# NagabhushanSN95/SimpleNeRF

Hardware: AMD Instinct MI355X
Metric: rays/sec (coarse+fine, 128+128 samples) (higher is better)
Workload: dtype f32; 1 GPU; headline: 1024 rays/GPU x (128 coarse + 128 fine -> 256 merged) samples, 8x256 coarse+fine MLPs, LLFF fern NDC rays, eval; rays_per_gpu=1024, samples=128+128, parallelism=ray-shard x1

## Files before the change

### simplenerf_amd/csrc/clock_stamp.h

```cpp
#pragma once
#ifdef SNERF_CLOCK_STAMP
#define SNERF_STAMP_DEFINE(name)                                                                                          \
    static __device__ unsigned long long name##_stamps[2 * 8192];                                                         \
    extern "C" __attribute__((weak)) int snerf_debug_clock_stamps_##name(unsigned long long* host, int pairs) {           \
        return (int)hipMemcpyFromSymbol(host, HIP_SYMBOL(name##_stamps), sizeof(unsigned long long) * 2 * (pairs < 8192 ? pairs : 8192)); \
    }
#define SNERF_STAMP_BEGIN() \
    const unsigned long long stamp_t0 = __builtin_amdgcn_s_memtime(), stamp_r0 = __builtin_amdgcn_s_memrealtime()
#define SNERF_STAMP_END(name)                                                                       \
    do {                                                                                            \
        if (threadIdx.x == 0) {                                                                     \
            name##_stamps[2 * (blockIdx.x & 8191)] = __builtin_amdgcn_s_memtime() - stamp_t0;       \
            name##_stamps[2 * (blockIdx.x & 8191) + 1] = __builtin_amdgcn_s_memrealtime() - stamp_r0; \
        }                                                                                           \
    } while (0)
#else
#define SNERF_STAMP_DEFINE(name)
#define SNERF_STAMP_BEGIN() do {} while (0)
#define SNERF_STAMP_END(name) do {} while (0)
#endif
```

### simplenerf_amd/csrc/composite.hip

```cpp
#include "composite_device.h"

namespace {

template <int C, bool RESAMPLE = false>
__global__ void __launch_bounds__(256) composite_kernel(CompositeArgs a) {
    extern __shared__ __attribute__((aligned(16))) float lds[];
    const int lane = snerf::lane_id();
    const long long ray = (long long)blockIdx.x * 4 + (threadIdx.x >> 6);
    if (ray >= a.num_rays) return;
    const int s = a.s;
    float* mine = RESAMPLE ? lds + (size_t)(threadIdx.x >> 6) * (s + snerf::resample_scratch_floats(s, a.s_f)) : nullptr;
    composite_ray<C, RESAMPLE>(a, ray, a.z + ray * s, a.sigma + ray * s, a.rgb + ray * s * 3, mine,
                               RESAMPLE ? a.z_fine + ray * (s + a.s_f) : nullptr, lane);
}

template <int C, bool RESAMPLE = false>
void launch(const CompositeArgs& a, hipStream_t stream) {
    const long long blocks = (a.num_rays + 3) / 4;
    const size_t lds_bytes = RESAMPLE ? 4 * sizeof(float) * (size_t)(a.s + snerf::resample_scratch_floats(a.s, a.s_f)) : 0;
    hipLaunchKernelGGL((composite_kernel<C, RESAMPLE>), dim3((unsigned)blocks), dim3(256), lds_bytes, stream, a);
}

template <bool RESAMPLE>
void launch_for_samples(const CompositeArgs& a, hipStream_t st) {
    const int c = (a.s + 63) / 64;
    switch (c) {
        case 1: launch<1, RESAMPLE>(a, st); break;
        case 2: launch<2, RESAMPLE>(a, st); break;
        case 3: launch<3, RESAMPLE>(a, st); break;
        case 4: launch<4, RESAMPLE>(a, st); break;
        case 5: case 6: launch<6, RESAMPLE>(a, st); break;
        case 7: case 8: launch<8, RESAMPLE>(a, st); break;
        default: launch<16, RESAMPLE>(a, st); break;
    }
}


struct CompositeBwdArgs {
    const float* sigma; const float* rgb; const float* z; const float* march_dirs; const float* rays_o; const float* rays_d;
    const float* g_rgb; const float* g_acc; const float* g_depth; const float* g_depth_ndc;
    float* d_sigma; float* d_rgb;
    long long num_rays; int s; int ndc; int white;
};

template <int C>
__global__ void __launch_bounds__(256) composite_backward_kernel(CompositeBwdArgs a) {
    const int lane = snerf::lane_id();
    const long long ray = (long long)blockIdx.x * 4 + (threadIdx.x >> 6);
    if (ray >= a.num_rays) return;
    const int s = a.s;
    const float* zr = a.z + ray * s;
    const float* sr = a.sigma + ray * s;
    const float* cr = a.rgb + ray * s * 3;
    const int j0 = lane * C;
    float z[C + 1], sg[C], col[C][3];
#pragma unroll
    for (int c = 0; c < C; ++c) {
        const int j = j0 + c;
        const bool in = j < s;
        z[c] = in ? zr[j] : 0.0f;
        sg[c] = in ? sr[j] : 0.0f;
#pragma unroll
        for (int k = 0; k < 3; ++k) col[c][k] = in ? cr[3 * j + k] : 0.0f;
    }
    const float far_cap = a.ndc ? 1.0f : 1e10f;
    z[C] = __shfl_down(z[0], 1, 64);
    if (j0 + C >= s) z[C] = far_cap;
#pragma unroll
    for (int c = 0; c < C; ++c)
        if (j0 + c == s - 1) z[c + 1] = far_cap;
    const float* md = a.march_dirs + ray * 3;
    const float norm = sqrtf((md[0] * md[0] + md[1] * md[1]) + md[2] * md[2]);

    float alpha[C], delta[C], keep = 1.0f;
#pragma unroll
    for (int c = 0; c < C; ++c) {
        const bool in = j0 + c < s;
        delta[c] = (z[c + 1] - z[c]) * norm;
        alpha[c] = in ? 1.0f - expf(-sg[c] * delta[c]) : 0.0f;
        keep *= in ? (1.0f - alpha[c]) + 1e-10f : 1.0f;
    }
    const float incl = snerf::wave_inclusive_mul(keep);
    float trans = __shfl_up(incl, 1, 64);
    if (lane == 0) trans = 1.0f;
    float T[C], w[C], acc = 0.0f, dzm = 0.0f;
#pragma unroll
    for (int c = 0; c < C; ++c) {
        T[c] = trans;
        w[c] = alpha[c] * trans;
        trans *= (1.0f - alpha[c]) + 1e-10f;
        acc += w[c];
        dzm += w[c] * z[c];
    }
    acc = snerf::wave_sum(acc);
    dzm = snerf::wave_sum(dzm);
    const float inv = __fdiv_rn(1.0f, acc + 1e-6f);
    const float depth_march = dzm * inv;
    float zd[C];
    float depth = depth_march;
    if (a.ndc) {
        const float oz = a.rays_o[ray * 3 + 2], dzw = a.rays_d[ray * 3 + 2];
        const float tn = __fdiv_rn(-(1.0f + oz), dzw);
        const float scale = __fdiv_rn(oz + tn * dzw, dzw);
        float dw = 0.0f;
#pragma unroll
        for (int c = 0; c < C; ++c) {
            const float cst = (z[c] == 1.0f) ? 1e-3f : 0.0f;
            zd[c] = scale * (__fdiv_rn(1.0f, (1.0f - z[c]) + cst) - 1.0f) + tn;
            dw += w[c] * zd[c];
        }
        depth = snerf::wave_sum(dw) * inv;
    } else {
#pragma unroll
        for (int c = 0; c < C; ++c) zd[c] = z[c];
    }
    const float gr = a.g_rgb ? a.g_rgb[ray * 3 + 0] : 0.0f;
    const float gg = a.g_rgb ? a.g_rgb[ray * 3 + 1] : 0.0f;
    const float gb = a.g_rgb ? a.g_rgb[ray * 3 + 2] : 0.0f;
    float gacc = a.g_acc ? a.g_acc[ray] : 0.0f;
    if (a.white) gacc -= (gr + gg) + gb;
    const float gdep = (a.g_depth ? a.g_depth[ray] : 0.0f) * inv;
    const float gdn = (a.ndc && a.g_depth_ndc ? a.g_depth_ndc[ray] : 0.0f) * inv;

    float g[C], local = 0.0f;
#pragma unroll
    for (int c = 0; c < C; ++c) {
        g[c] = ((gr * col[c][0] + gg * col[c][1]) + gb * col[c][2]) + gacc + gdep * (zd[c] - depth) + gdn * (z[c] - depth_march);
        local += g[c] * w[c];
    }
    const float suffix_incl = snerf::wave_suffix_add(local);
    float after = __shfl_down(suffix_incl, 1, 64);
    if (lane == 63) after = 0.0f;
#pragma unroll
    for (int c = C - 1; c >= 0; --c) {
        const int j = j0 + c;
        if (j < s) {
            const float u = (1.0f - alpha[c]) + 1e-10f;
            const float dalpha = g[c] * T[c] - __fdiv_rn(after, u);
            a.d_sigma[ray * s + j] = dalpha * (delta[c] * (1.0f - alpha[c]));
            a.d_rgb[(ray * s + j) * 3 + 0] = w[c] * gr;
            a.d_rgb[(ray * s + j) * 3 + 1] = w[c] * gg;
            a.d_rgb[(ray * s + j) * 3 + 2] = w[c] * gb;
        }
        after += g[c] * w[c];
    }
}

template <int C>
void launch_bwd(const CompositeBwdArgs& a, hipStream_t stream) {
    const long long blocks = (a.num_rays + 3) / 4;
    hipLaunchKernelGGL(composite_backward_kernel<C>, dim3((unsigned)blocks), dim3(256), 0, stream, a);
}

}

extern "C" int snerf_composite(const float* sigma, const float* rgb, const float* depths, const float* march_dirs,
                               const float* rays_o, const float* rays_d, long long num_rays, int num_samples, int ndc,
                               int white_bkgd, float* out_rgb, float* out_acc, float* out_alpha, float* out_visibility,
                               float* out_weights, float* out_depth, float* out_depth_var, float* out_depth_ndc,
                               float* out_depth_var_ndc, snerf_stream_t stream) {
    SNERF_REQUIRE(sigma && rgb && depths && march_dirs, "composite: NULL input");
    SNERF_REQUIRE(out_rgb && out_acc && out_depth && out_depth_var, "composite: NULL required output");
    SNERF_REQUIRE(!ndc || (rays_o && rays_d && out_depth_ndc && out_depth_var_ndc),
                  "composite: ndc needs world rays and the *_ndc outputs");
    SNERF_REQUIRE(num_rays >= 0 && num_samples >= 1, "composite: bad sizes n=%lld S=%d", num_rays, num_samples);
    if (num_samples > 64 * 16)
        return snerf::fail(SNERF_E_UNSUPPORTED, "composite: at most 1024 samples per ray (got %d)", num_samples);
    if (num_rays == 0) return SNERF_OK;
    if ((num_rays + 3) / 4 > 0x7fffffffLL) return snerf::fail(SNERF_E_UNSUPPORTED, "composite: too many rays in one call");
    CompositeArgs a{sigma, rgb, depths, march_dirs, rays_o, rays_d, out_rgb, out_acc, out_alpha, out_visibility,
                    out_weights, out_depth, out_depth_var, out_depth_ndc, out_depth_var_ndc, num_rays, num_samples,
                    ndc, white_bkgd, 0, nullptr, nullptr};
    launch_for_samples<false>(a, (hipStream_t)stream);
    return snerf::check_launch("composite");
}

namespace snerf {
int composite_resample(const float* sigma, const float* rgb, const float* depths, const float* march_dirs, const float* rays_o,
                       const float* rays_d, long long num_rays, int num_samples, int ndc, int white_bkgd, float* out_rgb,
                       float* out_acc, float* out_alpha, float* out_visibility, float* out_weights, float* out_depth,
                       float* out_depth_var, float* out_depth_ndc, float* out_depth_var_ndc, int num_fine, const float* u,
                       float* depths_fine, hipStream_t stream) {
    SNERF_REQUIRE(sigma && rgb && depths && march_dirs && depths_fine, "composite_resample: NULL input");
    SNERF_REQUIRE(out_rgb && out_acc && out_depth && out_depth_var, "composite_resample: NULL required output");
    SNERF_REQUIRE(!ndc || (rays_o && rays_d && out_depth_ndc && out_depth_var_ndc),
                  "composite_resample: ndc needs world rays and the *_ndc outputs");
    if (num_samples < 3 || num_fine < 1 || num_samples > 64 * 16 || (num_rays + 3) / 4 > 0x7fffffffLL ||
        4 * sizeof(float) * (size_t)(num_samples + resample_scratch_floats(num_samples, num_fine)) > 64 * 1024)
        return fail(SNERF_E_UNSUPPORTED, "composite_resample: %d + %d samples not built as one kernel", num_samples, num_fine);
    if (num_rays == 0) return SNERF_OK;
    CompositeArgs a{sigma, rgb, depths, march_dirs, rays_o, rays_d, out_rgb, out_acc, out_alpha, out_visibility,
                    out_weights, out_depth, out_depth_var, out_depth_ndc, out_depth_var_ndc, num_rays, num_samples,
                    ndc, white_bkgd, num_fine, u, depths_fine};
    launch_for_samples<true>(a, stream);
    return check_launch("composite_resample");
}
}

extern "C" int snerf_composite_backward(const float* sigma, const float* rgb, const float* depths, const float* march_dirs,
                                        const float* rays_o, const float* rays_d, long long num_rays, int num_samples,
                                        int ndc, int white_bkgd, const float* grad_rgb, const float* grad_acc,
                                        const float* grad_depth, const float* grad_depth_ndc, float* d_sigma, float* d_rgb,
                                        snerf_stream_t stream) {
    SNERF_REQUIRE(sigma && rgb && depths && march_dirs && d_sigma && d_rgb, "composite_backward: NULL pointer");
    SNERF_REQUIRE(!ndc || (rays_o && rays_d), "composite_backward: ndc needs the world rays");
    SNERF_REQUIRE(num_rays >= 0 && num_samples >= 1, "composite_backward: bad sizes n=%lld S=%d", num_rays, num_samples);
    if (num_samples > 64 * 16)
        return snerf::fail(SNERF_E_UNSUPPORTED, "composite_backward: at most 1024 samples per ray (got %d)", num_samples);
    if (num_rays == 0) return SNERF_OK;
    if ((num_rays + 3) / 4 > 0x7fffffffLL) return snerf::fail(SNERF_E_UNSUPPORTED, "composite_backward: too many rays");
    CompositeBwdArgs a{sigma, rgb, depths, march_dirs, rays_o, rays_d, grad_rgb, grad_acc, grad_depth, grad_depth_ndc,
                       d_sigma, d_rgb, num_rays, num_samples, ndc, white_bkgd};
    hipStream_t st = (hipStream_t)stream;
    const int c = (num_samples + 63) / 64;
    switch (c) {
        case 1: launch_bwd<1>(a, st); break;
        case 2: launch_bwd<2>(a, st); break;
        case 3: launch_bwd<3>(a, st); break;
        case 4: launch_bwd<4>(a, st); break;
        case 5: case 6: launch_bwd<6>(a, st); break;
        case 7: case 8: launch_bwd<8>(a, st); break;
        default: launch_bwd<16>(a, st); break;
    }
    return snerf::check_launch("composite_backward");
}
```

### simplenerf_amd/csrc/composite_device.h

```cpp
#pragma once
#include "resample_device.h"
#include "snerf_common.h"
#include "wave.h"

namespace {

struct CompositeArgs {
    const float* sigma; const float* rgb; const float* z; const float* march_dirs; const float* rays_o; const float* rays_d;
    float* out_rgb; float* out_acc; float* out_alpha; float* out_vis; float* out_weights;
    float* out_depth; float* out_depth_var; float* out_depth_ndc; float* out_depth_var_ndc;
    long long num_rays; int s; int ndc; int white;
    int s_f; const float* u; float* z_fine;
};

template <int C, bool RESAMPLE>
__device__ __forceinline__ void composite_ray(const CompositeArgs& a, long long ray, const float* zr, const float* sr,
                                              const float* cr, float* mine, float* z_fine, int lane) {
    const int s = a.s;
    const int j0 = lane * C;

    float z[C + 1], sg[C], col[C][3];
#pragma unroll
    for (int c = 0; c < C; ++c) {
        const int j = j0 + c;
        const bool in = j < s;
        z[c] = in ? zr[j] : 0.0f;
        sg[c] = in ? sr[j] : 0.0f;
#pragma unroll
        for (int k = 0; k < 3; ++k) col[c][k] = in ? cr[3 * j + k] : 0.0f;
    }
    const float far_cap = a.ndc ? 1.0f : 1e10f;
    z[C] = __shfl_down(z[0], 1, 64);
    if (j0 + C >= s) z[C] = far_cap;
#pragma unroll
    for (int c = 0; c < C; ++c)
        if (j0 + c == s - 1) z[c + 1] = far_cap;

    const float* md = a.march_dirs + ray * 3;
    const float norm = sqrtf((md[0] * md[0] + md[1] * md[1]) + md[2] * md[2]);

    float alpha[C], keep = 1.0f;
#pragma unroll
    for (int c = 0; c < C; ++c) {
        const bool in = j0 + c < s;
        const float delta = (z[c + 1] - z[c]) * norm;
        alpha[c] = in ? 1.0f - expf(-sg[c] * delta) : 0.0f;
        keep *= in ? (1.0f - alpha[c]) + 1e-10f : 1.0f;
    }
    const float incl = snerf::wave_inclusive_mul(keep);
    float trans = __shfl_up(incl, 1, 64);
    if (lane == 0) trans = 1.0f;

    float w[C], acc = 0.0f, r = 0.0f, g = 0.0f, b = 0.0f, dz = 0.0f;
#pragma unroll
    for (int c = 0; c < C; ++c) {
        const bool in = j0 + c < s;
        w[c] = alpha[c] * trans;
        if (in) {
            const int j = j0 + c;
            if (a.out_alpha) a.out_alpha[ray * s + j] = alpha[c];
            if (a.out_vis) a.out_vis[ray * s + j] = trans;
            if (a.out_weights) a.out_weights[ray * s + j] = w[c];
        }
        trans *= (1.0f - alpha[c]) + 1e-10f;
        acc += w[c];
        r += w[c] * col[c][0];
        g += w[c] * col[c][1];
        b += w[c] * col[c][2];
        dz += w[c] * z[c];
    }
    acc = snerf::wave_sum(acc);
    r = snerf::wave_sum(r);
    g = snerf::wave_sum(g);
    b = snerf::wave_sum(b);
    dz = snerf::wave_sum(dz);
    const float depth_march = __fdiv_rn(dz, acc + 1e-6f);
    float var = 0.0f;
#pragma unroll
    for (int c = 0; c < C; ++c) {
        const float d = z[c] - depth_march;
        var += w[c] * (d * d);
    }
    var = snerf::wave_sum(var);

    float depth = depth_march, depth_var = var;
    if (a.ndc) {
        const float oz = a.rays_o[ray * 3 + 2], dzw = a.rays_d[ray * 3 + 2];
        const float tn = __fdiv_rn(-(1.0f + oz), dzw);
        const float scale = __fdiv_rn(oz + tn * dzw, dzw);
        float zw[C], dw = 0.0f;
#pragma unroll
        for (int c = 0; c < C; ++c) {
            const float cst = (z[c] == 1.0f) ? 1e-3f : 0.0f;
            zw[c] = scale * (__fdiv_rn(1.0f, (1.0f - z[c]) + cst) - 1.0f) + tn;
            dw += w[c] * zw[c];
        }
        dw = snerf::wave_sum(dw);
        depth = __fdiv_rn(dw, acc + 1e-6f);
        float vw = 0.0f;
#pragma unroll
        for (int c = 0; c < C; ++c) {
            const float d = zw[c] - depth;
            vw += w[c] * (d * d);
        }
        depth_var = snerf::wave_sum(vw);
    }
    if (lane == 0) {
        if (a.white) {
            const float bg = 1.0f - acc;
            r += bg; g += bg; b += bg;
        }
        a.out_rgb[ray * 3 + 0] = r;
        a.out_rgb[ray * 3 + 1] = g;
        a.out_rgb[ray * 3 + 2] = b;
        a.out_acc[ray] = acc;
        a.out_depth[ray] = depth;
        a.out_depth_var[ray] = depth_var;
        if (a.ndc) {
            a.out_depth_ndc[ray] = depth_march;
            a.out_depth_var_ndc[ray] = var;
        }
    }
    if constexpr (RESAMPLE) {
#pragma unroll
        for (int c = 0; c < C; ++c)
            if (j0 + c < s) mine[j0 + c] = w[c];
        snerf::wave_lds_sync();
        snerf::resample_wave(zr, mine, s, a.s_f, a.u ? a.u + ray * a.s_f : nullptr, z_fine, mine + s, lane);
    }
}

}
```

### simplenerf_amd/csrc/resample_device.h

```cpp
#pragma once
#include "wave.h"

namespace snerf {

__device__ __forceinline__ float unit_linspace(int i, int steps) {
    if (steps == 1) return 0.0f;
    const float step = __fdiv_rn(1.0f, (float)(steps - 1));
    return (i < steps / 2) ? fmaf(step, (float)i, 0.0f) : fmaf(-step, (float)(steps - 1 - i), 1.0f);
}

__device__ __forceinline__ float torch_row_sum(const float* __restrict__ w, int n, int lane) {
    const int width = n >= 8 ? 8 : 1;
    const int l = width == 8 ? (lane & 7) : 0;
    const int vectors = n / width;
    const int groups = vectors / 4;
    int level_power = 4;
    {
        int lg = 1;
        if (groups > 2) lg = 32 - __clz(groups - 1);
        if (lg / 4 > level_power) level_power = lg / 4;
    }
    const int level_step = 1 << level_power;
    const int level_mask = level_step - 1;
    float acc[4][4];
#pragma unroll
    for (int j = 0; j < 4; ++j)
#pragma unroll
        for (int k = 0; k < 4; ++k) acc[j][k] = 0.0f;
    auto at = [&](int vec) { return w[vec * width + l] + 1e-5f; };
    int i = 0;
    for (; i + level_step <= groups;) {
        for (int j = 0; j < level_step; ++j, ++i)
#pragma unroll
            for (int k = 0; k < 4; ++k) acc[0][k] += at(i * 4 + k);
#pragma unroll
        for (int j = 1; j < 4; ++j) {
#pragma unroll
            for (int k = 0; k < 4; ++k) { acc[j][k] += acc[j - 1][k]; acc[j - 1][k] = 0.0f; }
            if ((i & (level_mask << (j * level_power))) != 0) break;
        }
    }
    for (; i < groups; ++i)
#pragma unroll
        for (int k = 0; k < 4; ++k) acc[0][k] += at(i * 4 + k);
#pragma unroll
    for (int j = 1; j < 4; ++j)
#pragma unroll
        for (int k = 0; k < 4; ++k) acc[0][k] += acc[j][k];
    float lane_sum = acc[0][0];
    for (int v = groups * 4; v < vectors; ++v) lane_sum += at(v);
    lane_sum += acc[0][1];
    lane_sum += acc[0][2];
    lane_sum += acc[0][3];
    if (width == 1) return lane_sum;
    float total = 0.0f;
    for (int k = vectors * 8; k < n; ++k) total += w[k] + 1e-5f;
#pragma unroll
    for (int k = 0; k < 8; ++k) total += __shfl(lane_sum, k, 64);
    return total;
}

__host__ __device__ inline int resample_scratch_floats(int s_c, int s_f) { return (s_c + s_f) + 2 * (s_c - 1); }

__device__ __forceinline__ void resample_wave(const float* __restrict__ zc, const float* __restrict__ wc, int s_c, int s_f,
                                              const float* __restrict__ u, float* __restrict__ out, float* scratch, int lane) {
    const int total = s_c + s_f;
    const int nb = s_c - 1;
    const int m = s_c - 2;
    float* merged = scratch;
    float* cdf = merged + total;
    float* bins = cdf + nb;

    for (int j = lane; j < s_c; j += 64) merged[j] = zc[j];
    snerf::wave_lds_sync();
    for (int j = lane; j < nb; j += 64) bins[j] = 0.5f * (merged[j + 1] + merged[j]);

    const float denom_sum = torch_row_sum(wc + 1, m, lane);
    if (lane == 0) cdf[0] = 0.0f;
    double run = 0.0;
    for (int base = 0; base < m; base += 64) {
        const int j = base + lane;
        const float mine = j < m ? __fdiv_rn(wc[j + 1] + 1e-5f, denom_sum) : 0.0f;
        const int count = m - base < 64 ? m - base : 64;
        float entry = 0.0f;
        for (int k = 0; k < count; ++k) {
            run += (double)__builtin_bit_cast(float, __builtin_amdgcn_readlane(__builtin_bit_cast(int, mine), k));
            if (lane == k) entry = (float)run;
        }
        if (j < m) cdf[j + 1] = entry;
    }
    snerf::wave_lds_sync();

    for (int k = lane; k < s_f; k += 64) {
        const float uk = u ? u[k] : unit_linspace(k, s_f);
        int lo = 0, hi = nb;
        while (lo < hi) {
            const int mid = (lo + hi) >> 1;
            if (cdf[mid] <= uk) lo = mid + 1; else hi = mid;
        }
        const int below = lo - 1 > 0 ? lo - 1 : 0;
        const int above = lo < nb - 1 ? lo : nb - 1;
        const float cb = cdf[below], ca = cdf[above];
        float den = ca - cb;
        if (den < 1e-5f) den = 1.0f;
        const float t = __fdiv_rn(uk - cb, den);
        const float bb = bins[below], ba = bins[above];
        merged[s_c + k] = bb + t * (ba - bb);
    }
    snerf::wave_lds_sync();

    const float* smp = merged + s_c;
    const bool sorted_samples = (u == nullptr);
    for (int j = lane; j < s_c; j += 64) {
        const float v = merged[j];
        int below;
        if (sorted_samples) {
            int lo = 0, hi = s_f;
            while (lo < hi) { const int mid = (lo + hi) >> 1; if (smp[mid] < v) lo = mid + 1; else hi = mid; }
            below = lo;
        } else {
            below = 0;
            for (int q = 0; q < s_f; ++q) below += smp[q] < v;
        }
        out[j + below] = v;
    }
    for (int k = lane; k < s_f; k += 64) {
        const float v = smp[k];
        int lo = 0, hi = s_c;
        while (lo < hi) { const int mid = (lo + hi) >> 1; if (merged[mid] <= v) lo = mid + 1; else hi = mid; }
        int among = k;
        if (!sorted_samples) {
            among = 0;
            for (int q = 0; q < s_f; ++q) { const float x = smp[q]; among += (x < v) || (x == v && q < k); }
        }
        out[lo + among] = v;
    }
}

}
```

Before: 312,100 rays/s.

## Parallelize resample CDF scan with DPP and pair binary searches

The serial 64-step readlane prefix sum over CDF weights is replaced by a DPP-based double-precision inclusive scan. It is used only when a range check shows the double sums are exact, and otherwise falls back to the old serial loop. Binary searches for inverse-CDF sampling and for the merge now handle two elements per lane at once, which raises instruction-level parallelism. Coarse z values are staged into LDS from registers instead of reloaded from global memory, u values are prefetched early, and phase timing stamps are added that compile out by default.

```diff
diff --git a/simplenerf_amd/csrc/clock_stamp.h b/simplenerf_amd/csrc/clock_stamp.h
--- a/simplenerf_amd/csrc/clock_stamp.h
+++ b/simplenerf_amd/csrc/clock_stamp.h
@@ -14,7 +14,24 @@
             name##_stamps[2 * (blockIdx.x & 8191) + 1] = __builtin_amdgcn_s_memrealtime() - stamp_r0; \
         }                                                                                           \
     } while (0)
+static __device__ unsigned long long snerf_phase_stamps[16 * 1024];
+#define SNERF_PHASE(k, after)                                                                          \
+    do {                                                                                               \
+        asm volatile("" ::"v"(after) : "memory");                                                      \
+        if (threadIdx.x == 0 && blockIdx.x < 1024) snerf_phase_stamps[blockIdx.x * 16 + (k)] = __builtin_amdgcn_s_memtime(); \
+    } while (0)
+#define SNERF_PHASE_REAL(k)                                                                            \
+    do {                                                                                               \
+        if (threadIdx.x == 0 && blockIdx.x < 1024) snerf_phase_stamps[blockIdx.x * 16 + (k)] = __builtin_amdgcn_s_memrealtime(); \
+    } while (0)
+#define SNERF_PHASES_ACCESSOR(name)                                                                    \
+    extern "C" int snerf_debug_phase_stamps_##name(unsigned long long* host, int groups) {             \
+        return (int)hipMemcpyFromSymbol(host, HIP_SYMBOL(snerf_phase_stamps), sizeof(unsigned long long) * 16 * (groups < 1024 ? groups : 1024)); \
+    }
 #else
+#define SNERF_PHASE(k, after) do {} while (0)
+#define SNERF_PHASE_REAL(k) do {} while (0)
+#define SNERF_PHASES_ACCESSOR(name)
 #define SNERF_STAMP_DEFINE(name)
 #define SNERF_STAMP_BEGIN() do {} while (0)
 #define SNERF_STAMP_END(name) do {} while (0)
diff --git a/simplenerf_amd/csrc/composite.hip b/simplenerf_amd/csrc/composite.hip
--- a/simplenerf_amd/csrc/composite.hip
+++ b/simplenerf_amd/csrc/composite.hip
@@ -1,4 +1,6 @@
 #include "composite_device.h"
+
+SNERF_PHASES_ACCESSOR(composite)
 
 namespace {
 
diff --git a/simplenerf_amd/csrc/composite_device.h b/simplenerf_amd/csrc/composite_device.h
--- a/simplenerf_amd/csrc/composite_device.h
+++ b/simplenerf_amd/csrc/composite_device.h
@@ -18,6 +18,7 @@
                                               const float* cr, float* mine, float* z_fine, int lane) {
     const int s = a.s;
     const int j0 = lane * C;
+    if constexpr (RESAMPLE) { SNERF_PHASE_REAL(14); SNERF_PHASE(0, lane); }
 
     float z[C + 1], sg[C], col[C][3];
 #pragma unroll
@@ -38,6 +39,8 @@
 
     const float* md = a.march_dirs + ray * 3;
     const float norm = sqrtf((md[0] * md[0] + md[1] * md[1]) + md[2] * md[2]);
+    const float oz = a.ndc ? a.rays_o[ray * 3 + 2] : 0.0f, dzw = a.ndc ? a.rays_d[ray * 3 + 2] : 0.0f;
+    if constexpr (RESAMPLE) SNERF_PHASE(1, (((z[0] + sg[0]) + col[0][0]) + col[0][1]) + (col[0][2] + norm));
 
     float alpha[C], keep = 1.0f;
 #pragma unroll
@@ -85,7 +88,6 @@
 
     float depth = depth_march, depth_var = var;
     if (a.ndc) {
-        const float oz = a.rays_o[ray * 3 + 2], dzw = a.rays_d[ray * 3 + 2];
         const float tn = __fdiv_rn(-(1.0f + oz), dzw);
         const float scale = __fdiv_rn(oz + tn * dzw, dzw);
         float zw[C], dw = 0.0f;
@@ -105,6 +107,7 @@
         }
         depth_var = snerf::wave_sum(vw);
     }
+    if constexpr (RESAMPLE) SNERF_PHASE(2, depth_var + depth);
     if (lane == 0) {
         if (a.white) {
             const float bg = 1.0f - acc;
@@ -124,9 +127,10 @@
     if constexpr (RESAMPLE) {
 #pragma unroll
         for (int c = 0; c < C; ++c)
-            if (j0 + c < s) mine[j0 + c] = w[c];
+            if (j0 + c < s) { mine[j0 + c] = w[c]; mine[s + j0 + c] = z[c]; }
         snerf::wave_lds_sync();
-        snerf::resample_wave(zr, mine, s, a.s_f, a.u ? a.u + ray * a.s_f : nullptr, z_fine, mine + s, lane);
+        snerf::resample_wave(mine + s, mine, s, a.s_f, a.u ? a.u + ray * a.s_f : nullptr, z_fine, mine + s, lane);
+        SNERF_PHASE_REAL(15);
     }
 }
 
diff --git a/simplenerf_amd/csrc/resample_device.h b/simplenerf_amd/csrc/resample_device.h
--- a/simplenerf_amd/csrc/resample_device.h
+++ b/simplenerf_amd/csrc/resample_device.h
@@ -1,4 +1,5 @@
 #pragma once
+#include "clock_stamp.h"
 #include "wave.h"
 
 namespace snerf {
@@ -62,6 +63,48 @@
 
 __host__ __device__ inline int resample_scratch_floats(int s_c, int s_f) { return (s_c + s_f) + 2 * (s_c - 1); }
 
+template <bool UPPER>
+__device__ __forceinline__ void search_pair(const float* a, int n, float va, float vb, int& ra, int& rb) {
+    int lo_a = 0, hi_a = n, lo_b = 0, hi_b = n;
+    while ((lo_a < hi_a) | (lo_b < hi_b)) {
+        const int mid_a = (lo_a + hi_a) >> 1, mid_b = (lo_b + hi_b) >> 1;
+        const float xa = a[mid_a < n ? mid_a : n - 1], xb = a[mid_b < n ? mid_b : n - 1];
+        const bool up_a = UPPER ? xa <= va : xa < va, up_b = UPPER ? xb <= vb : xb < vb;
+        if (lo_a < hi_a) { if (up_a) lo_a = mid_a + 1; else hi_a = mid_a; }
+        if (lo_b < hi_b) { if (up_b) lo_b = mid_b + 1; else hi_b = mid_b; }
+    }
+    ra = lo_a;
+    rb = lo_b;
+}
+
+__device__ __forceinline__ float inverse_cdf_sample(const float* cdf, const float* bins, int nb, int idx, float uk) {
+    const int below = idx - 1 > 0 ? idx - 1 : 0;
+    const int above = idx < nb - 1 ? idx : nb - 1;
+    const float cb = cdf[below], ca = cdf[above];
+    float den = ca - cb;
+    if (den < 1e-5f) den = 1.0f;
+    const float t = __fdiv_rn(uk - cb, den);
+    const float bb = bins[below], ba = bins[above];
+    return bb + t * (ba - bb);
+}
+
+template <int CTRL, int ROW_MASK>
+__device__ __forceinline__ double dpp_move_or_zero(double v) {
+    const unsigned long long bits = __builtin_bit_cast(unsigned long long, v);
+    const int lo = __builtin_amdgcn_update_dpp(0, (int)(unsigned)bits, CTRL, ROW_MASK, 0xf, false);
+    const int hi = __builtin_amdgcn_update_dpp(0, (int)(unsigned)(bits >> 32), CTRL, ROW_MASK, 0xf, false);
+    return __builtin_bit_cast(double, ((unsigned long long)(unsigned)hi << 32) | (unsigned)lo);
+}
+__device__ __forceinline__ double wave_inclusive_add_exact(double v) {
+    v += dpp_move_or_zero<0x111, 0xf>(v);
+    v += dpp_move_or_zero<0x112, 0xf>(v);
+    v += dpp_move_or_zero<0x114, 0xf>(v);
+    v += dpp_move_or_zero<0x118, 0xf>(v);
+    v += dpp_move_or_zero<0x142, 0xa>(v);
+    v += dpp_move_or_zero<0x143, 0xc>(v);
+    return v;
+}
+
 __device__ __forceinline__ void resample_wave(const float* __restrict__ zc, const float* __restrict__ wc, int s_c, int s_f,
                                               const float* __restrict__ u, float* __restrict__ out, float* scratch, int lane) {
     const int total = s_c + s_f;
@@ -71,70 +114,118 @@
     float* cdf = merged + total;
     float* bins = cdf + nb;
 
-    for (int j = lane; j < s_c; j += 64) merged[j] = zc[j];
+    float u_first = 0.0f, u_second = 0.0f;
+    if (u) {
+        if (lane < s_f) u_first = u[lane];
+        if (lane + 64 < s_f) u_second = u[lane + 64];
+    }
+    if (zc != merged) {
+        for (int j = lane; j < s_c; j += 64) merged[j] = zc[j];
+        snerf::wave_lds_sync();
+    }
+    for (int j = lane; j < nb; j += 64) bins[j] = 0.5f * (merged[j + 1] + merged[j]);
+    SNERF_PHASE(3, lane);
+
+    const float denom_sum = torch_row_sum(wc + 1, m, lane);
+    SNERF_PHASE(4, denom_sum);
+    if (lane == 0) cdf[0] = 0.0f;
+    float largest = 0.0f, smallest = __builtin_inff();
+    bool plain = true;
+    for (int j = lane; j < m; j += 64) {
+        const float mine = __fdiv_rn(wc[j + 1] + 1e-5f, denom_sum);
+        cdf[j + 1] = mine;
+        plain = plain && mine >= 0.0f && mine < __builtin_inff();
+        largest = fmaxf(largest, mine);
+        if (mine > 0.0f) smallest = fminf(smallest, mine);
+    }
+#pragma unroll
+    for (int off = 32; off > 0; off >>= 1) {
+        largest = fmaxf(largest, __shfl_xor(largest, off, 64));
+        smallest = fminf(smallest, __shfl_xor(smallest, off, 64));
+    }
+    bool exact = __all(plain);
+    if (exact && largest > 0.0f) {
+        const double bound_sum = (double)m * (double)largest;
+        const int e = (int)((__builtin_bit_cast(unsigned long long, bound_sum) >> 52) & 0x7ff) - 1023 + 1;
+        const double least = __builtin_bit_cast(double, (unsigned long long)(e - 29 + 1023) << 52);
+        exact = e - 29 + 1023 > 0 && (double)smallest >= least;
+    }
+    if (exact) {
+        double carry = 0.0;
+        for (int base = 0; base < m; base += 64) {
+            const int j = base + lane;
+            const double sum = carry + wave_inclusive_add_exact(j < m ? (double)cdf[j + 1] : 0.0);
+            if (j < m) cdf[j + 1] = (float)sum;
+            const unsigned long long bits = __builtin_bit_cast(unsigned long long, sum);
+            carry = __builtin_bit_cast(double, ((unsigned long long)(unsigned)__builtin_amdgcn_readlane((int)(unsigned)(bits >> 32), 63) << 32) |
+                                                   (unsigned)__builtin_amdgcn_readlane((int)(unsigned)bits, 63));
+        }
+    } else {
+        double run = 0.0;
+        for (int base = 0; base < m; base += 64) {
+            const int j = base + lane;
+            const float mine = j < m ? cdf[j + 1] : 0.0f;
+            const int count = m - base < 64 ? m - base : 64;
+            float entry = 0.0f;
+            for (int k = 0; k < count; ++k) {
+                run += (double)__builtin_bit_cast(float, __builtin_amdgcn_readlane(__builtin_bit_cast(int, mine), k));
+                if (lane == k) entry = (float)run;
+            }
+            if (j < m) cdf[j + 1] = entry;
+        }
+    }
     snerf::wave_lds_sync();
-    for (int j = lane; j < nb; j += 64) bins[j] = 0.5f * (merged[j + 1] + merged[j]);
-
-    const float denom_sum = torch_row_sum(wc + 1, m, lane);
-    if (lane == 0) cdf[0] = 0.0f;
-    double run = 0.0;
-    for (int base = 0; base < m; base += 64) {
-        const int j = base + lane;
-        const float mine = j < m ? __fdiv_rn(wc[j + 1] + 1e-5f, denom_sum) : 0.0f;
-        const int count = m - base < 64 ? m - base : 64;
-        float entry = 0.0f;
-        for (int k = 0; k < count; ++k) {
-            run += (double)__builtin_bit_cast(float, __builtin_amdgcn_readlane(__builtin_bit_cast(int, mine), k));
-            if (lane == k) entry = (float)run;
-        }
-        if (j < m) cdf[j + 1] = entry;
+    SNERF_PHASE(5, lane);
+
+    for (int k = lane; k < s_f; k += 128) {
+        const int k2 = k + 64;
+        const bool two = k2 < s_f;
+        const float uk = u ? (k == lane ? u_first : u[k]) : unit_linspace(k, s_f);
+        const float uk2 = !two ? uk : u ? (k == lane ? u_second : u[k2]) : unit_linspace(k2, s_f);
+        int idx, idx2;
+        search_pair<true>(cdf, nb, uk, uk2, idx, idx2);
+        merged[s_c + k] = inverse_cdf_sample(cdf, bins, nb, idx, uk);
+        if (two) merged[s_c + k2] = inverse_cdf_sample(cdf, bins, nb, idx2, uk2);
     }
     snerf::wave_lds_sync();
-
-    for (int k = lane; k < s_f; k += 64) {
-        const float uk = u ? u[k] : unit_linspace(k, s_f);
-        int lo = 0, hi = nb;
-        while (lo < hi) {
-            const int mid = (lo + hi) >> 1;
-            if (cdf[mid] <= uk) lo = mid + 1; else hi = mid;
-        }
-        const int below = lo - 1 > 0 ? lo - 1 : 0;
-        const int above = lo < nb - 1 ? lo : nb - 1;
-        const float cb = cdf[below], ca = cdf[above];
-        float den = ca - cb;
-        if (den < 1e-5f) den = 1.0f;
-        const float t = __fdiv_rn(uk - cb, den);
-        const float bb = bins[below], ba = bins[above];
-        merged[s_c + k] = bb + t * (ba - bb);
-    }
-    snerf::wave_lds_sync();
+    SNERF_PHASE(6, lane);
 
     const float* smp = merged + s_c;
     const bool sorted_samples = (u == nullptr);
-    for (int j = lane; j < s_c; j += 64) {
-        const float v = merged[j];
-        int below;
+    for (int j = lane; j < s_c; j += 128) {
+        const int j2 = j + 64;
+        const bool two = j2 < s_c;
+        const float v = merged[j], v2 = two ? merged[j2] : v;
+        int below, below2;
         if (sorted_samples) {
-            int lo = 0, hi = s_f;
-            while (lo < hi) { const int mid = (lo + hi) >> 1; if (smp[mid] < v) lo = mid + 1; else hi = mid; }
-            below = lo;
+            search_pair<false>(smp, s_f, v, v2, below, below2);
         } else {
-            below = 0;
-            for (int q = 0; q < s_f; ++q) below += smp[q] < v;
+            below = 0, below2 = 0;
+            for (int q = 0; q < s_f; ++q) { const float x = smp[q]; below += x < v; below2 += x < v2; }
         }
         out[j + below] = v;
-    }
-    for (int k = lane; k < s_f; k += 64) {
-        const float v = smp[k];
-        int lo = 0, hi = s_c;
-        while (lo < hi) { const int mid = (lo + hi) >> 1; if (merged[mid] <= v) lo = mid + 1; else hi = mid; }
-        int among = k;
+        if (two) out[j2 + below2] = v2;
+    }
+    SNERF_PHASE(7, lane);
+    for (int k = lane; k < s_f; k += 128) {
+        const int k2 = k + 64;
+        const bool two = k2 < s_f;
+        const float v = smp[k], v2 = two ? smp[k2] : v;
+        int lo, lo2;
+        search_pair<true>(merged, s_c, v, v2, lo, lo2);
+        int among = k, among2 = k2;
         if (!sorted_samples) {
-            among = 0;
-            for (int q = 0; q < s_f; ++q) { const float x = smp[q]; among += (x < v) || (x == v && q < k); }
+            among = 0, among2 = 0;
+            for (int q = 0; q < s_f; ++q) {
+                const float x = smp[q];
+                among += (x < v) || (x == v && q < k);
+                among2 += (x < v2) || (x == v2 && q < k2);
+            }
         }
         out[lo + among] = v;
-    }
-}
-
-}
+        if (two) out[lo2 + among2] = v2;
+    }
+    SNERF_PHASE(8, lane);
+}
+
+}
```

After: 313,800 rays/s (median of 5 runs). Within noise of the previous version (+0.5%).
